# RicherMans/PLDA

Measured on AMD Instinct MI355X. Metric: PLDA LLR trials/sec, higher is better.
Workload: dtype f32; 1 GPU; C2: 100k i-vectors, featdim 200, 5k speakers; 100k x 100k trials, n = 1; fit 10 EM iters; D_eff=200; enrol_models=100000, test_vectors=100000, parallelism=one GPU, score_dtype=f32 (fp64 bias terms, fp32 MFMA contraction), fit_dtype=f64

## Files before the change

### plda_amd/csrc/eer.hip

```cpp
#include "trial_source.hpp"

#include <algorithm>
#include <cstring>

namespace plda {


typedef float f32x4e __attribute__((ext_vector_type(4)));

__global__ __launch_bounds__(256) void eer_hist_kernel(const float *__restrict__ scores, int64_t Nt, int fixed_class,
                                                       int shift, int nbits, unsigned prefix, int has_prefix,
                                                       unsigned long long *__restrict__ hist ,
                                                       unsigned *__restrict__ below, unsigned *__restrict__ above) {
  __shared__ unsigned lh[2][EER_BINS];
  for (int i = threadIdx.x; i < 2 * EER_BINS; i += 256) (&lh[0][0])[i] = 0;
  __syncthreads();
  const unsigned mask = (1u << nbits) - 1u;
  const int hi_shift = shift + nbits;
  unsigned lo_max = 0u, hi_min = 0xffffffffu;

  auto account = [&](bool ok, float sc, int cls) {
    unsigned bin = 0xffffffffu;
    if (ok) {
      const unsigned k = score_key(sc);
      if (has_prefix && (k >> hi_shift) != prefix) {
        if ((k >> hi_shift) < prefix) lo_max = k > lo_max ? k : lo_max; else hi_min = k < hi_min ? k : hi_min;
      } else {
        bin = ((k >> shift) & mask) | ((unsigned)cls << 11);
      }
    }
    if (bin != 0xffffffffu) atomicAdd(&lh[bin >> 11][bin & 2047u], 1u);
  };

  for (int64_t idx = (int64_t)blockIdx.x * 256 + threadIdx.x; idx - threadIdx.x < Nt; idx += (int64_t)gridDim.x * 256)
    account(idx < Nt, idx < Nt ? scores[idx] : 0.f, fixed_class);
  __syncthreads();
  for (int i = threadIdx.x; i < 2 * EER_BINS; i += 256) {
    const unsigned v = (&lh[0][0])[i];
    if (v) atomicAdd(hist + i, (unsigned long long)v);
  }
  if (has_prefix) {
    if (lo_max) atomicMax(below, lo_max);
    if (hi_min != 0xffffffffu) atomicMin(above, hi_min);
  }
}

__global__ __launch_bounds__(256) void eer_hist_strip_kernel(const float *__restrict__ scores, int64_t ld, int64_t M,
                                                             int64_t Nt, const int64_t *__restrict__ espk,
                                                             const int64_t *__restrict__ tspk, int64_t rows_per_wg,
                                                             int shift, int nbits, unsigned prefix, int has_prefix,
                                                             unsigned long long *__restrict__ hist,
                                                             unsigned *__restrict__ below, unsigned *__restrict__ above, int64_t row_step) {
  __shared__ unsigned lh[2][EER_BINS];
  for (int i = threadIdx.x; i < 2 * EER_BINS; i += 256) (&lh[0][0])[i] = 0;
  __syncthreads();
  const unsigned mask = (1u << nbits) - 1u;
  const int hi_shift = shift + nbits;
  unsigned lo_max = 0u, hi_min = 0xffffffffu;
  const int64_t strips = (Nt + EER_STRIP - 1) / EER_STRIP;
  const int64_t strip = blockIdx.x % strips, slice = blockIdx.x / strips;
  const int64_t col = strip * EER_STRIP + (int64_t)threadIdx.x * 4;
  const int64_t r0 = slice * rows_per_wg, r1 = (r0 + rows_per_wg < M) ? r0 + rows_per_wg : M;
  int64_t ts[4];
  bool ok[4];
#pragma unroll
  for (int e = 0; e < 4; ++e) {
    ok[e] = col + e < Nt;
    ts[e] = ok[e] ? tspk[col + e] : 0;
  }
  const bool vec = ((ld & 3) == 0) && ((reinterpret_cast<uintptr_t>(scores) & 15) == 0) && ok[3];

  auto account = [&](float sc, int cls) {
    const unsigned k = score_key(sc);
    if (has_prefix && (k >> hi_shift) != prefix) {
      if ((k >> hi_shift) < prefix) lo_max = k > lo_max ? k : lo_max; else hi_min = k < hi_min ? k : hi_min;
    } else {
      atomicAdd(&lh[cls][(k >> shift) & mask], 1u);
    }
  };

  for (int64_t row = r0; row < r1; row += 4) {
    float v[4][4];
#pragma unroll
    for (int u = 0; u < 4; ++u) {
      if (row + u >= r1) break;
      const float *src = scores + (row + u) * row_step * ld + col;
      if (vec) {
        const f32x4e x = __builtin_nontemporal_load(reinterpret_cast<const f32x4e *>(src));
        v[u][0] = x.x; v[u][1] = x.y; v[u][2] = x.z; v[u][3] = x.w;
      } else {
#pragma unroll
        for (int e = 0; e < 4; ++e) v[u][e] = ok[e] ? src[e] : 0.f;
      }
    }
#pragma unroll
    for (int u = 0; u < 4; ++u) {
      if (row + u >= r1) break;
      const int64_t spk = espk[(row + u) * row_step];
#pragma unroll
      for (int e = 0; e < 4; ++e) if (ok[e]) account(v[u][e], ts[e] == spk ? 1 : 0);
    }
  }
  __syncthreads();
  for (int i = threadIdx.x; i < 2 * EER_BINS; i += 256) {
    const unsigned c = (&lh[0][0])[i];
    if (c) atomicAdd(hist + i, (unsigned long long)c);
  }
  if (has_prefix) {
    if (lo_max) atomicMax(below, lo_max);
    if (hi_min != 0xffffffffu) atomicMin(above, hi_min);
  }
}

struct EerWindowOut {
  unsigned long long below[2], targets, above, cursor[2];
};
constexpr int EER_WBUF = 1536;
__global__ __launch_bounds__(256) void eer_window_strip_kernel(const float *__restrict__ scores, int64_t ld, int64_t M, int64_t Nt,
                                                               const int64_t *__restrict__ espk, const int64_t *__restrict__ tspk,
                                                               int64_t rows_per_wg, float flo, float fhi, EerWindowOut *__restrict__ wo,
                                                               float *__restrict__ list0, float *__restrict__ list1, unsigned long long cap) {
  __shared__ unsigned long long red[4][4];
  __shared__ float stage[4][2][EER_WBUF];
  __shared__ int fillc[4][2];
  const int64_t strips = (Nt + EER_STRIP - 1) / EER_STRIP;
  const int64_t strip = blockIdx.x % strips, slice = blockIdx.x / strips;
  const int64_t col = strip * EER_STRIP + (int64_t)threadIdx.x * 4;
  const int64_t r0 = slice * rows_per_wg, r1 = (r0 + rows_per_wg < M) ? r0 + rows_per_wg : M;
  const int lane = threadIdx.x & 63, wave = threadIdx.x >> 6;
  int64_t ts[4];
  bool ok[4];
#pragma unroll
  for (int e = 0; e < 4; ++e) {
    ok[e] = col + e < Nt;
    ts[e] = ok[e] ? tspk[col + e] : 0;
  }
  const bool vec = ((ld & 3) == 0) && ((reinterpret_cast<uintptr_t>(scores) & 15) == 0) && ok[3];
  const float qnan = __uint_as_float(0x7fc00000u);
  unsigned b0 = 0, b1 = 0, t1 = 0, ab = 0;
  int *const fc = fillc[wave];
  if (lane < 2) fc[lane] = 0;
  auto flush = [&](int c) {
    const int n = __builtin_amdgcn_readfirstlane(fc[c]);
    if (n == 0) return;
    unsigned long long base = 0;
    if (lane == 0) base = atomicAdd(&wo->cursor[c], (unsigned long long)n);
    base = __shfl(base, 0);
    float *dst = c ? list1 : list0;
    const float *src = stage[wave][c];
    for (int i = lane; i < n; i += 64)
      if (base + i < cap) dst[base + i] = src[i];
    if (lane == 0) fc[c] = 0;
  };
  for (int64_t row = r0; row < r1; row += 4) {
    float v[4][4];
#pragma unroll
    for (int u = 0; u < 4; ++u) {
      if (row + u >= r1) break;
      const float *src = scores + (row + u) * ld + col;
      if (vec) {
        const f32x4e x = __builtin_nontemporal_load(reinterpret_cast<const f32x4e *>(src));
        v[u][0] = x.x; v[u][1] = x.y; v[u][2] = x.z; v[u][3] = x.w;
      } else {
#pragma unroll
        for (int e = 0; e < 4; ++e) v[u][e] = ok[e] ? src[e] : qnan;
      }
    }
#pragma unroll
    for (int u = 0; u < 4; ++u) {
      if (row + u >= r1) break;
      const int64_t spk = espk[row + u];
#pragma unroll
      for (int e = 0; e < 4; ++e) {
        const float x = v[u][e];
        const bool tgt = ok[e] && ts[e] == spk;
        const bool lt_lo = x < flo, lt_hi = x < fhi;
        t1 += tgt ? 1u : 0u;
        b1 += (lt_lo && tgt) ? 1u : 0u;
        b0 += (lt_lo && !tgt) ? 1u : 0u;
        ab += (x >= fhi) ? 1u : 0u;
        if (lt_hi && !lt_lo) {
          const int c = tgt ? 1 : 0;
          const int slot = atomicAdd(&fc[c], 1);
          stage[wave][c][slot] = x;
        }
      }
    }
    if (__builtin_amdgcn_readfirstlane(fc[0]) > EER_WBUF - 1024) flush(0);
    if (__builtin_amdgcn_readfirstlane(fc[1]) > EER_WBUF - 1024) flush(1);
  }
  flush(0);
  flush(1);
  unsigned long long c[4] = {b0, b1, t1, ab};
#pragma unroll
  for (int q = 0; q < 4; ++q) {
    for (int o = 32; o > 0; o >>= 1) c[q] += __shfl_xor(c[q], o);
    if (lane == 0) red[wave][q] = c[q];
  }
  __syncthreads();
  if (threadIdx.x < 4) {
    const unsigned long long sum = (red[0][threadIdx.x] + red[1][threadIdx.x]) + (red[2][threadIdx.x] + red[3][threadIdx.x]);
    unsigned long long *dst = threadIdx.x == 0 ? &wo->below[0] : threadIdx.x == 1 ? &wo->below[1] : threadIdx.x == 2 ? &wo->targets : &wo->above;
    if (sum) atomicAdd(dst, sum);
  }
}


int eer_pass(plda_handle *h, const TrialSource &src, int shift, int nbits, unsigned prefix, int has_prefix,
             unsigned long long *dhist, unsigned *dbelow, unsigned *dabove, std::vector<unsigned long long> &hh) {
  PLDA_HIP(h, hipMemsetAsync(dhist, 0, 2 * EER_BINS * 8, h->stream));
  PLDA_TRY(for_each_piece(src, [&](const TrialPiece &pc) -> int {
    if (pc.cls < 0) {
      const int64_t strips = ceil_div(pc.Nt, (int64_t)EER_STRIP);
      const int64_t slices = std::max<int64_t>(1, std::min<int64_t>(pc.rows, (256 * 16) / strips));
      const int64_t rows_per_wg = ceil_div(pc.rows, slices);
      eer_hist_strip_kernel<<<(unsigned)(strips * ceil_div(pc.rows, rows_per_wg)), 256, 0, h->stream>>>(
          pc.scores, pc.ld, pc.rows, pc.Nt, pc.espk, src.tspk, rows_per_wg, shift, nbits, prefix, has_prefix, dhist, dbelow, dabove,
          pc.row_step);
    } else {
      const unsigned grid = (unsigned)std::min<int64_t>(ceil_div(pc.Nt, 256), 256 * 16);
      eer_hist_kernel<<<grid, 256, 0, h->stream>>>(pc.scores, pc.Nt, pc.cls, shift, nbits, prefix, has_prefix, dhist, dbelow, dabove);
    }
    return PLDA_OK;
  }));
  PLDA_LAUNCH_CHECK(h);
  hh.resize(2 * EER_BINS);
  PLDA_HIP(h, hipMemcpyAsync(hh.data(), dhist, 2 * EER_BINS * 8, hipMemcpyDeviceToHost, h->stream));
  PLDA_HIP(h, hipStreamSynchronize(h->stream));
  return PLDA_OK;
}

bool reduce_block_or_poison(plda_handle *h, const TrialSource &src, const char *who, unsigned long long *H, int *rc) {
  constexpr unsigned long long POISON = 1ull << 48;
  if (src.reduce) {
    if (*rc != PLDA_OK) { std::fill(H, H + 2 * EER_BINS, 0ull); H[0] = POISON; }
    if (src.reduce(src.ctx, H, nullptr, nullptr) != 0 && *rc == PLDA_OK) *rc = fail(h, PLDA_E_INVAL, "%s: the caller's reduction failed", who);
    if (*rc == PLDA_OK && H[0] >= POISON) *rc = fail(h, PLDA_E_NUMERIC, "%s: another rank of the sharded call failed", who);
  }
  return *rc == PLDA_OK;
}

static int eer_device(plda_handle *h, const TrialSource &src, double *out, bool *window_missed = nullptr) {
  typedef unsigned __int128 u128;
  if (window_missed) *window_missed = false;
  unsigned long long *dhist;
  unsigned *dbelow;
  PLDA_TRY(carve(h, h->trial_hist, [&](Layout &c) { c.take(dhist, 2 * EER_BINS).take(dbelow, 2).slack(56); }));
  unsigned *dabove = dbelow + 1;
  std::vector<unsigned long long> H;
  unsigned long long Np = 0, Nn = 0, Pb = 0, Nb = 0;
  unsigned prefix = 0;
  const int shifts[3] = {21, 10, 0}, bits[3] = {11, 11, 10};
  unsigned long long cP = 0, cN = 0;
  std::vector<unsigned long long> last;
  static const unsigned init[2] = {0u, 0xffffffffu};
  int rc = PLDA_OK;
  for (int pass = 0; pass < 3; ++pass) {
    if (rc == PLDA_OK && pass == 2) {
      const hipError_t e = hipMemcpyAsync(dbelow, init, 8, hipMemcpyHostToDevice, h->stream);
      if (e != hipSuccess) rc = hip_fail(h, e, "hipMemcpyAsync(dbelow)", __FILE__, __LINE__);
    }
    if (rc == PLDA_OK) rc = eer_pass(h, src, shifts[pass], bits[pass], prefix, pass > 0, dhist, dbelow, dabove, H);
    H.resize(2 * EER_BINS);
    if (!reduce_block_or_poison(h, src, "eer", H.data(), &rc)) continue;
    const int nb = 1 << bits[pass];
    if (pass == 0) {
      for (int b = 0; b < nb; ++b) { Nn += H[b]; Np += H[EER_BINS + b]; }
      if (src.windowed) { Np = src.tot_p; Nn = src.tot_n; Pb = src.base_p; Nb = src.base_n; }
      if (Np == 0 || Nn == 0) { rc = fail(h, PLDA_E_INVAL, "eer: need at least one target and one impostor trial"); continue; }
    }
    int sel = -1;
    unsigned long long P = Pb, N = Nb;
    for (int b = 0; b < nb; ++b) {
      const unsigned long long p2 = P + H[EER_BINS + b], n2 = N + H[b];
      if ((H[b] | H[EER_BINS + b]) && (u128)p2 * Nn >= (u128)(Nn - n2) * Np) { sel = b; cP = H[EER_BINS + b]; cN = H[b]; break; }
      P = p2; N = n2;
    }
    if (sel < 0 && src.windowed && window_missed) { *window_missed = true; return PLDA_OK; }
    if (sel < 0) { rc = fail(h, PLDA_E_NUMERIC, "eer: crossing not found (inconsistent counts)"); continue; }
    Pb = P; Nb = N;
    prefix = (prefix << bits[pass]) | (unsigned)sel;
    if (pass == 2) last = H;
  }
  unsigned hb[2] = {0u, 0xffffffffu};
  if (rc == PLDA_OK) {
    hipError_t e = hipMemcpyAsync(hb, dbelow, 8, hipMemcpyDeviceToHost, h->stream);
    if (e == hipSuccess) e = hipStreamSynchronize(h->stream);
    if (e != hipSuccess) rc = hip_fail(h, e, "copy of the neighbour keys", __FILE__, __LINE__);
  }
  if (src.reduce && src.reduce(src.ctx, nullptr, &hb[0], &hb[1]) != 0 && rc == PLDA_OK)
    rc = fail(h, PLDA_E_INVAL, "eer: the caller's reduction failed");
  if (rc != PLDA_OK) return rc;
  const unsigned k1 = prefix;
  const int b2 = (int)(k1 & 1023u);
  long long k0 = -1, k2 = -1;
  for (int b = b2 - 1; b >= 0; --b) if (last[b] | last[EER_BINS + b]) { k0 = (long long)((k1 & ~1023u) | (unsigned)b); break; }
  if (k0 < 0 && (Pb + Nb) > 0) k0 = hb[0];
  for (int b = b2 + 1; b < 1024; ++b) if (last[b] | last[EER_BINS + b]) { k2 = (long long)((k1 & ~1023u) | (unsigned)b); break; }
  if (k2 < 0 && (Pb + cP + Nb + cN) < (Np + Nn)) k2 = hb[1];
  if (src.windowed) {
    const bool need0 = (Pb + Nb) > 0, need2 = (Pb + cP + Nb + cN) < (Np + Nn);
    if ((need0 && k0 == 0) || (need2 && k2 == 0xffffffffll)) { if (window_missed) *window_missed = true; return PLDA_OK; }
  }
  const double far1 = (double)(Nn - Nb - cN) / (double)Nn, frr1 = (double)(Pb + cP) / (double)Np;
  const double far0 = (double)(Nn - Nb) / (double)Nn, frr0 = (double)Pb / (double)Np;
  double thr, far, frr;
  if (fabs(far1 - frr1) <= fabs(far0 - frr0)) {
    const double s = key_score(k1);
    thr = k2 >= 0 ? s + ((double)key_score((unsigned)k2) - s) / 2.0 : s + 1e-8;
    far = (double)(Nn - Nb - cN) / (double)Nn; frr = (double)(Pb + cP) / (double)Np;
  } else {
    const double s1 = key_score(k1);
    thr = k0 >= 0 ? (double)key_score((unsigned)k0) + (s1 - (double)key_score((unsigned)k0)) / 2.0 : s1;
    far = (double)(Nn - Nb) / (double)Nn; frr = (double)Pb / (double)Np;
  }
  out[0] = thr; out[1] = far; out[2] = frr; out[3] = 0.5 * (far + frr); out[4] = (double)Np; out[5] = (double)Nn;
  return PLDA_OK;
}

constexpr int64_t EER_PILOT_STEP = 32;
static int eer_matrix_windowed(plda_handle *h, const TrialSource &full, double *out, bool *done) {
  typedef unsigned __int128 u128;
  *done = false;
  const int64_t M = full.M, Nt = full.Nt;
  TraceScope ts(h, "eer.pilot");
  unsigned long long *dhist;
  unsigned *dbelow;
  EerWindowOut *dwo;
  PLDA_TRY(carve(h, h->trial_hist, [&](Layout &c) { c.take(dhist, 2 * EER_BINS).take(dbelow, 2).take(dwo, 1, 64); }));
  unsigned *dabove = dbelow + 1;
  TrialSource smp = TrialSource::matrix(full.scores, full.ld, M, Nt, full.espk, full.tspk).every(EER_PILOT_STEP);
  int64_t pilot_step = EER_PILOT_STEP;
  if (full.kind == TrialSource::SLABS) {
    pilot_step = std::max<int64_t>(EER_PILOT_STEP, ceil_div(M, full.sl->slab_rows));
    const float *sc = nullptr; const int64_t *se = nullptr; int64_t sld = 0, srows = 0;
    PLDA_TRY(full.sl->sample(full.sl->ctx, pilot_step, &sc, &sld, &se, &srows));
    smp = TrialSource::matrix(sc, sld, srows, Nt, se, full.tspk);
  }
  std::vector<unsigned long long> H0, H1;
  PLDA_TRY(eer_pass(h, smp, 21, 11, 0, 0, dhist, dbelow, dabove, H0));
  unsigned long long Np = 0, Nn = 0;
  for (int b = 0; b < EER_BINS; ++b) { Nn += H0[b]; Np += H0[EER_BINS + b]; }
  if (Np < 2000 || Nn < 2000) return PLDA_OK;
  auto g_after = [&](unsigned long long p, unsigned long long n) { return (double)p / (double)Np - (double)(Nn - n) / (double)Nn; };
  double delta = 0.0;
  {
    unsigned long long P = 0, N = 0;
    int c0 = -1;
    for (int b = 0; b < EER_BINS; ++b) {
      const unsigned long long p2 = P + H0[EER_BINS + b], n2 = N + H0[b];
      if ((H0[b] | H0[EER_BINS + b]) && (u128)p2 * Nn >= (u128)(Nn - n2) * Np) { c0 = b; break; }
      P = p2; N = n2;
    }
    if (c0 < 0) return PLDA_OK;
    const double pe = std::min(0.5, std::max((double)P / (double)Np, 10.0 / (double)Np));
    delta = 5.0 * (std::sqrt(pe * (1.0 - pe) / (double)Np) + std::sqrt(pe * (1.0 - pe) / (double)Nn)) + 2.0 / (double)Np;
  }
  int ca = -1, cb = -1;
  unsigned long long Pa = 0, Na = 0, Pc = 0, Nc = 0;
  {
    unsigned long long P = 0, N = 0;
    for (int b = 0; b < EER_BINS; ++b) {
      const unsigned long long p2 = P + H0[EER_BINS + b], n2 = N + H0[b];
      const double g = g_after(p2, n2);
      if (ca < 0 && g > -delta) { ca = b; Pa = P; Na = N; }
      if (g >= delta) { cb = b; Pc = P; Nc = N; break; }
      P = p2; N = n2;
    }
  }
  if (ca < 0 || cb < 0) return PLDA_OK;
  int blo = 0, bhi = EER_BINS - 1;
  unsigned long long win_lo = Pa + Na, win_hi = 0;
  PLDA_TRY(eer_pass(h, smp, 10, 11, (unsigned)ca, 1, dhist, dbelow, dabove, H1));
  {
    unsigned long long p = Pa, n = Na;
    for (int b = 0; b < EER_BINS; ++b) {
      const unsigned long long p2 = p + H1[EER_BINS + b], n2 = n + H1[b];
      if (g_after(p2, n2) > -delta) { blo = b; break; }
      p = p2; n = n2;
    }
    blo = std::max(blo - 1, 0);
    for (int b = 0; b < blo; ++b) win_lo += H1[b] + H1[EER_BINS + b];
  }
  if (cb != ca) PLDA_TRY(eer_pass(h, smp, 10, 11, (unsigned)cb, 1, dhist, dbelow, dabove, H1));
  {
    unsigned long long p = Pc, n = Nc;
    for (int b = 0; b < EER_BINS; ++b) {
      p += H1[EER_BINS + b]; n += H1[b];
      if (g_after(p, n) >= delta) { bhi = b; break; }
    }
    bhi = std::min(bhi + 1, EER_BINS - 1);
    win_hi = Pc + Nc;
    for (int b = 0; b <= bhi; ++b) win_hi += H1[b] + H1[EER_BINS + b];
  }
  const unsigned klo = ((unsigned)ca << 21) | ((unsigned)blo << 10);
  const unsigned long long khi64 = ((unsigned long long)cb << 21) | ((unsigned long long)(bhi + 1) << 10);
  if (khi64 > 0xffffffffull || khi64 <= klo) return PLDA_OK;
  const unsigned khi = (unsigned)khi64;
  const unsigned long long win = win_hi > win_lo ? win_hi - win_lo : 0;
  const unsigned long long cap = (unsigned long long)((double)win * (double)pilot_step * 2.0) + (1ull << 20);
  if (cap > (unsigned long long)M * (unsigned long long)Nt / 8) return PLDA_OK;
  PLDA_HIP(h, h->eer_list[0].reserve((size_t)cap * 4));
  PLDA_HIP(h, h->eer_list[1].reserve((size_t)cap * 4));
  ts.next("eer.window_pass", (double)M * (double)Nt * 4.0, 2);
  PLDA_HIP(h, hipMemsetAsync(dwo, 0, sizeof(EerWindowOut), h->stream));
  PLDA_TRY(for_each_piece(full, [&](const TrialPiece &pc) -> int {
    const int64_t strips = ceil_div(Nt, (int64_t)EER_STRIP);
    const int64_t slices = std::max<int64_t>(1, std::min<int64_t>(pc.rows, (256 * 16) / strips));
    const int64_t rows_per_wg = ceil_div(pc.rows, slices);
    eer_window_strip_kernel<<<(unsigned)(strips * ceil_div(pc.rows, rows_per_wg)), 256, 0, h->stream>>>(
        pc.scores, pc.ld, pc.rows, Nt, pc.espk, full.tspk, rows_per_wg, key_score(klo), key_score(khi), dwo, h->eer_list[0].as<float>(), h->eer_list[1].as<float>(), cap);
    PLDA_LAUNCH_CHECK(h);
    return PLDA_OK;
  }));
  EerWindowOut wo;
  PLDA_HIP(h, hipMemcpyAsync(&wo, dwo, sizeof(wo), hipMemcpyDeviceToHost, h->stream));
  PLDA_HIP(h, hipStreamSynchronize(h->stream));
  ts.next("eer.finish_on_window");
  if (wo.cursor[0] > cap || wo.cursor[1] > cap) return PLDA_OK;
  if (wo.below[0] + wo.below[1] + wo.cursor[0] + wo.cursor[1] + wo.above != (unsigned long long)M * (unsigned long long)Nt) return PLDA_OK;
  const unsigned long long TP = wo.targets, TN = (unsigned long long)M * (unsigned long long)Nt - wo.targets;
  if (TP == 0 || TN == 0) return fail(h, PLDA_E_INVAL, "eer: need at least one target and one impostor trial");
  if ((u128)wo.below[1] * TN >= (u128)(TN - wo.below[0]) * TP) return PLDA_OK;
  if ((u128)(wo.below[1] + wo.cursor[1]) * TN < (u128)(TN - wo.below[0] - wo.cursor[0]) * TP) return PLDA_OK;
  if (wo.cursor[0] + wo.cursor[1] == 0) return PLDA_OK;
  const TrialSource lst = TrialSource::lists(h->eer_list[1].as<float>(), (int64_t)wo.cursor[1], h->eer_list[0].as<float>(), (int64_t)wo.cursor[0])
                              .window_of(wo.below[1], wo.below[0], TP, TN);
  bool missed = false;
  PLDA_TRY(eer_device(h, lst, out, &missed));
  *done = !missed;
  return PLDA_OK;
}

static int eer_source_device(plda_handle *h, const TrialSource &src, double *out, const char *three_passes_scope) {
  const int64_t M = src.M, Nt = src.Nt;
  h->eer_last_passes = 3;
  if (!src.reduce && h->eer_variant != 1 && (h->eer_variant == 2 || (double)M * (double)Nt >= 2.5e8) && M >= 4 * EER_PILOT_STEP) {
    bool done = false;
    PLDA_TRY(eer_matrix_windowed(h, src, out, &done));
    if (done) { h->eer_last_passes = 1; return PLDA_OK; }
  }
  TraceScope ts(h, three_passes_scope, 3.0 * (double)M * (double)Nt * 4.0, 2);
  return eer_device(h, src, out);
}

int eer_matrix_device(plda_handle *h, const float *dscores, int64_t ld, int64_t M, int64_t Nt, const int64_t *despk,
                      const int64_t *dtspk, double *out, TrialReduce reduce, void *ctx) {
  if (!out || Nt <= 0 || ld < Nt || M < 0 || (M == 0 && !reduce) || (M > 0 && (!dscores || !despk || !dtspk)))
    return fail(h, PLDA_E_INVAL, "eer: bad argument");
  return eer_source_device(h, TrialSource::matrix(dscores, ld, M, Nt, despk, dtspk).reduced_by(reduce, ctx), out, "eer.three_passes");
}

int score_eer_device(plda_handle *h, const double *dU, const int32_t *dn, int n_uniform, int64_t M, const double *dV, int64_t Nt,
                     const double *dzmean, const double *dzstd, const int64_t *despk, const int64_t *dtspk, double *out) {
  OperandSlabs os;
  TrialSource src;
  PLDA_TRY(operand_source(h, "score_eer", dU, dn, n_uniform, M, dV, Nt, dzmean, dzstd, despk, dtspk, out, &os, &src));
  return eer_source_device(h, src, out, "eer.three_passes (slabs re-scored per pass)");
}

constexpr int DET_MAX = 2047;
__global__ __launch_bounds__(256) void det_minmax_kernel(const float *__restrict__ scores, int64_t ld, int64_t M, int64_t Nt,
                                                         unsigned *__restrict__ mm ) {
  unsigned lo = 0xffffffffu, hi = 0u;
  const int64_t total = M * Nt;
  for (int64_t idx = (int64_t)blockIdx.x * 256 + threadIdx.x; idx < total; idx += (int64_t)gridDim.x * 256) {
    const unsigned k = score_key(scores[(idx / Nt) * ld + idx % Nt]);
    lo = k < lo ? k : lo; hi = k > hi ? k : hi;
  }
  for (int o = 32; o > 0; o >>= 1) {
    const unsigned a = __shfl_xor(lo, o), b = __shfl_xor(hi, o);
    lo = a < lo ? a : lo; hi = b > hi ? b : hi;
  }
  if ((threadIdx.x & 63) == 0) { atomicMin(mm, lo); atomicMax(mm + 1, hi); }
}
__global__ __launch_bounds__(256) void det_hist_kernel(const float *__restrict__ scores, int64_t ld, int64_t M, int64_t Nt,
                                                       const int64_t *__restrict__ espk, const int64_t *__restrict__ tspk, int cls,
                                                       const double *__restrict__ thr, int n, double lo, double inv_step,
                                                       unsigned long long *__restrict__ hist ) {
  __shared__ unsigned lh[2][DET_MAX + 1];
  __shared__ double ts[DET_MAX + 1];
  for (int i = threadIdx.x; i < 2 * (DET_MAX + 1); i += 256) (&lh[0][0])[i] = 0;
  for (int i = threadIdx.x; i < n; i += 256) ts[i] = thr[i];
  __syncthreads();
  const int64_t total = M * Nt;
  for (int64_t idx = (int64_t)blockIdx.x * 256 + threadIdx.x; idx < total; idx += (int64_t)gridDim.x * 256) {
    const int64_t r = idx / Nt, c = idx % Nt;
    const double sc = (double)scores[r * ld + c];
    int k = (int)((sc - lo) * inv_step) + 1;
    k = k < 0 ? 0 : (k > n ? n : k);
    while (k > 0 && ts[k - 1] > sc) --k;
    while (k < n && ts[k] <= sc) ++k;
    const int cl = cls >= 0 ? cls : (espk[r] == tspk[c] ? 1 : 0);
    atomicAdd(&lh[cl][k], 1u);
  }
  __syncthreads();
  for (int i = threadIdx.x; i < 2 * (DET_MAX + 1); i += 256) {
    const unsigned v = (&lh[0][0])[i];
    if (v) atomicAdd(hist + i, (unsigned long long)v);
  }
}

static int det_device(plda_handle *h, const TrialSource &src, int npoints, double *far, double *frr, double *thresholds) {
  if (npoints < 2 || npoints > DET_MAX) return fail(h, PLDA_E_INVAL, "det: 2 <= n_points <= %d", DET_MAX);
  const size_t hb = (size_t)2 * (DET_MAX + 1) * 8;
  unsigned long long *dhist;
  unsigned *dmm;
  double *dthr;
  PLDA_TRY(carve(h, h->trial_hist, [&](Layout &c) { c.take(dhist, 2 * (DET_MAX + 1)).take(dmm, 16).take(dthr, DET_MAX).slack(64); }));
  static const unsigned init[2] = {0xffffffffu, 0u};
  PLDA_HIP(h, hipMemcpyAsync(dmm, init, 8, hipMemcpyHostToDevice, h->stream));
  PLDA_TRY(for_each_piece(src, [&](const TrialPiece &pc) -> int {
    det_minmax_kernel<<<(unsigned)std::min<int64_t>(ceil_div(pc.rows * pc.Nt, 256), 256 * 32), 256, 0, h->stream>>>(pc.scores, pc.ld, pc.rows, pc.Nt, dmm);
    return PLDA_OK;
  }));
  PLDA_LAUNCH_CHECK(h);
  unsigned mm[2];
  PLDA_HIP(h, hipMemcpyAsync(mm, dmm, 8, hipMemcpyDeviceToHost, h->stream));
  PLDA_HIP(h, hipStreamSynchronize(h->stream));
  if (mm[0] > mm[1]) return fail(h, PLDA_E_INVAL, "det: no scores");
  const double lo = (double)key_score(mm[0]), hi = (double)key_score(mm[1]);
  const double step = (hi - lo) / ((double)npoints - 1.0);
  std::vector<double> thr((size_t)npoints);
  double t = lo;
  for (int i = 0; i < npoints; ++i) { thr[(size_t)i] = t; t += step; }
  PLDA_HIP(h, hipMemcpyAsync(dthr, thr.data(), (size_t)npoints * 8, hipMemcpyHostToDevice, h->stream));
  PLDA_HIP(h, hipMemsetAsync(dhist, 0, hb, h->stream));
  PLDA_TRY(for_each_piece(src, [&](const TrialPiece &pc) -> int {
    det_hist_kernel<<<(unsigned)std::min<int64_t>(ceil_div(pc.rows * pc.Nt, 256), 256 * 8), 256, 0, h->stream>>>(
        pc.scores, pc.ld, pc.rows, pc.Nt, pc.espk, src.tspk, pc.cls, dthr, npoints, lo, step > 0.0 ? 1.0 / step : 0.0, dhist);
    return PLDA_OK;
  }));
  PLDA_LAUNCH_CHECK(h);
  std::vector<unsigned long long> H((size_t)2 * (DET_MAX + 1));
  PLDA_HIP(h, hipMemcpyAsync(H.data(), dhist, hb, hipMemcpyDeviceToHost, h->stream));
  PLDA_HIP(h, hipStreamSynchronize(h->stream));
  unsigned long long Nn = 0, Np = 0;
  for (int k = 0; k <= npoints; ++k) { Nn += H[(size_t)k]; Np += H[(size_t)(DET_MAX + 1) + k]; }
  if (Nn == 0 || Np == 0) return fail(h, PLDA_E_INVAL, "det: need at least one target and one impostor score");
  unsigned long long below_p = 0, ge_n = Nn;
  for (int i = 0; i < npoints; ++i) {
    ge_n -= H[(size_t)i];
    below_p += H[(size_t)(DET_MAX + 1) + i];
    far[i] = (double)ge_n / (double)Nn;
    frr[i] = (double)below_p / (double)Np;
    if (thresholds) thresholds[i] = thr[(size_t)i];
  }
  return PLDA_OK;
}

int det_matrix_device(plda_handle *h, const float *dscores, int64_t ld, int64_t M, int64_t Nt, const int64_t *despk, const int64_t *dtspk,
                      int npoints, double *far, double *frr, double *thresholds) {
  if (!dscores || !despk || !dtspk || !far || !frr || M <= 0 || Nt <= 0 || ld < Nt) return fail(h, PLDA_E_INVAL, "det: bad argument");
  return det_device(h, TrialSource::matrix(dscores, ld, M, Nt, despk, dtspk), npoints, far, frr, thresholds);
}
int det_lists_device(plda_handle *h, const float *dpos, int64_t np, const float *dneg, int64_t nn, int npoints, double *far, double *frr,
                     double *thresholds) {
  if (!dpos || !dneg || !far || !frr || np <= 0 || nn <= 0) return fail(h, PLDA_E_INVAL, "det: need at least one target and one impostor score");
  return det_device(h, TrialSource::lists(dpos, np, dneg, nn), npoints, far, frr, thresholds);
}

int eer_lists_device(plda_handle *h, const float *dpos, int64_t np, const float *dneg, int64_t nn, double *out) {
  if (!dpos || !dneg || !out || np <= 0 || nn <= 0) return fail(h, PLDA_E_INVAL, "eer: need at least one target and one impostor score");
  return eer_device(h, TrialSource::lists(dpos, np, dneg, nn), out);
}

}
```

Before: 363.7 billion trials/s.

## Move windowed EER refinement on-device and rebalance window pass with persistent grid

The window pass becomes a persistent kernel sized to resident occupancy, with fixed row-chunk work units spread evenly over blocks. LDS stage-slot atomics are replaced by wave ballots and prefix popcounts. The per-pass host readback in the windowed list refinement is replaced by a single-block device scan kernel that chains the three histogram passes and reads back once. Neighbour min/max atomics are reduced per wave and skipped when they cannot change the stored value. This removes host sync round-trips and contention, at the cost of more kernel complexity and a smaller staging buffer that flushes more often.

```diff
diff --git a/plda_amd/csrc/eer.hip b/plda_amd/csrc/eer.hip
--- a/plda_amd/csrc/eer.hip
+++ b/plda_amd/csrc/eer.hip
@@ -7,14 +7,29 @@
 
 
 typedef float f32x4e __attribute__((ext_vector_type(4)));
+
+__device__ __forceinline__ void neighbours_to_global(unsigned lo_max, unsigned hi_min, unsigned *__restrict__ below,
+                                                     unsigned *__restrict__ above) {
+  for (int o = 32; o > 0; o >>= 1) {
+    const unsigned a = __shfl_xor(lo_max, o), b = __shfl_xor(hi_min, o);
+    lo_max = a > lo_max ? a : lo_max;
+    hi_min = b < hi_min ? b : hi_min;
+  }
+  if ((threadIdx.x & 63) == 0) {
+    if (lo_max > __hip_atomic_load(below, __ATOMIC_RELAXED, __HIP_MEMORY_SCOPE_AGENT)) atomicMax(below, lo_max);
+    if (hi_min < __hip_atomic_load(above, __ATOMIC_RELAXED, __HIP_MEMORY_SCOPE_AGENT)) atomicMin(above, hi_min);
+  }
+}
 
 __global__ __launch_bounds__(256) void eer_hist_kernel(const float *__restrict__ scores, int64_t Nt, int fixed_class,
                                                        int shift, int nbits, unsigned prefix, int has_prefix,
                                                        unsigned long long *__restrict__ hist ,
-                                                       unsigned *__restrict__ below, unsigned *__restrict__ above) {
+                                                       unsigned *__restrict__ below, unsigned *__restrict__ above,
+                                                       const unsigned *__restrict__ dprefix = nullptr) {
   __shared__ unsigned lh[2][EER_BINS];
   for (int i = threadIdx.x; i < 2 * EER_BINS; i += 256) (&lh[0][0])[i] = 0;
   __syncthreads();
+  if (dprefix) prefix = *dprefix;
   const unsigned mask = (1u << nbits) - 1u;
   const int hi_shift = shift + nbits;
   unsigned lo_max = 0u, hi_min = 0xffffffffu;
@@ -39,10 +54,7 @@
     const unsigned v = (&lh[0][0])[i];
     if (v) atomicAdd(hist + i, (unsigned long long)v);
   }
-  if (has_prefix) {
-    if (lo_max) atomicMax(below, lo_max);
-    if (hi_min != 0xffffffffu) atomicMin(above, hi_min);
-  }
+  if (has_prefix) neighbours_to_global(lo_max, hi_min, below, above);
 }
 
 __global__ __launch_bounds__(256) void eer_hist_strip_kernel(const float *__restrict__ scores, int64_t ld, int64_t M,
@@ -106,42 +118,30 @@
     const unsigned c = (&lh[0][0])[i];
     if (c) atomicAdd(hist + i, (unsigned long long)c);
   }
-  if (has_prefix) {
-    if (lo_max) atomicMax(below, lo_max);
-    if (hi_min != 0xffffffffu) atomicMin(above, hi_min);
-  }
+  if (has_prefix) neighbours_to_global(lo_max, hi_min, below, above);
 }
 
 struct EerWindowOut {
   unsigned long long below[2], targets, above, cursor[2];
 };
-constexpr int EER_WBUF = 1536;
+constexpr int EER_WROWS = 8;
+constexpr int EER_WROW_MAX = 256;
+constexpr int EER_WBUF = 512;
+static_assert(EER_WBUF >= 2 * EER_WROW_MAX, "a row must fit the stage behind the flush threshold");
 __global__ __launch_bounds__(256) void eer_window_strip_kernel(const float *__restrict__ scores, int64_t ld, int64_t M, int64_t Nt,
                                                                const int64_t *__restrict__ espk, const int64_t *__restrict__ tspk,
-                                                               int64_t rows_per_wg, float flo, float fhi, EerWindowOut *__restrict__ wo,
-                                                               float *__restrict__ list0, float *__restrict__ list1, unsigned long long cap) {
-  __shared__ unsigned long long red[4][4];
+                                                               int64_t chunks, int64_t units, float flo, float fhi, EerWindowOut *__restrict__ wo,
+                                                               float *__restrict__ list0, float *__restrict__ list1, unsigned long long cap,
+                                                               unsigned long long *__restrict__ hist_clear) {
   __shared__ float stage[4][2][EER_WBUF];
-  __shared__ int fillc[4][2];
-  const int64_t strips = (Nt + EER_STRIP - 1) / EER_STRIP;
-  const int64_t strip = blockIdx.x % strips, slice = blockIdx.x / strips;
-  const int64_t col = strip * EER_STRIP + (int64_t)threadIdx.x * 4;
-  const int64_t r0 = slice * rows_per_wg, r1 = (r0 + rows_per_wg < M) ? r0 + rows_per_wg : M;
+  if (hist_clear && blockIdx.x == 0)
+    for (int i = threadIdx.x; i < 2 * EER_BINS; i += 256) hist_clear[i] = 0ull;
   const int lane = threadIdx.x & 63, wave = threadIdx.x >> 6;
-  int64_t ts[4];
-  bool ok[4];
-#pragma unroll
-  for (int e = 0; e < 4; ++e) {
-    ok[e] = col + e < Nt;
-    ts[e] = ok[e] ? tspk[col + e] : 0;
-  }
-  const bool vec = ((ld & 3) == 0) && ((reinterpret_cast<uintptr_t>(scores) & 15) == 0) && ok[3];
+  const unsigned long long lower = (1ull << lane) - 1ull;
   const float qnan = __uint_as_float(0x7fc00000u);
-  unsigned b0 = 0, b1 = 0, t1 = 0, ab = 0;
-  int *const fc = fillc[wave];
-  if (lane < 2) fc[lane] = 0;
-  auto flush = [&](int c) {
-    const int n = __builtin_amdgcn_readfirstlane(fc[c]);
+  unsigned wlo = 0, wlo1 = 0, wt = 0, wab = 0;
+  int fill0 = 0, fill1 = 0;
+  auto flush = [&](int c, int n) {
     if (n == 0) return;
     unsigned long long base = 0;
     if (lane == 0) base = atomicAdd(&wo->cursor[c], (unsigned long long)n);
@@ -150,56 +150,73 @@
     const float *src = stage[wave][c];
     for (int i = lane; i < n; i += 64)
       if (base + i < cap) dst[base + i] = src[i];
-    if (lane == 0) fc[c] = 0;
   };
-  for (int64_t row = r0; row < r1; row += 4) {
-    float v[4][4];
-#pragma unroll
-    for (int u = 0; u < 4; ++u) {
-      if (row + u >= r1) break;
-      const float *src = scores + (row + u) * ld + col;
-      if (vec) {
-        const f32x4e x = __builtin_nontemporal_load(reinterpret_cast<const f32x4e *>(src));
-        v[u][0] = x.x; v[u][1] = x.y; v[u][2] = x.z; v[u][3] = x.w;
-      } else {
-#pragma unroll
-        for (int e = 0; e < 4; ++e) v[u][e] = ok[e] ? src[e] : qnan;
-      }
-    }
-#pragma unroll
-    for (int u = 0; u < 4; ++u) {
-      if (row + u >= r1) break;
-      const int64_t spk = espk[row + u];
-#pragma unroll
-      for (int e = 0; e < 4; ++e) {
-        const float x = v[u][e];
-        const bool tgt = ok[e] && ts[e] == spk;
-        const bool lt_lo = x < flo, lt_hi = x < fhi;
-        t1 += tgt ? 1u : 0u;
-        b1 += (lt_lo && tgt) ? 1u : 0u;
-        b0 += (lt_lo && !tgt) ? 1u : 0u;
-        ab += (x >= fhi) ? 1u : 0u;
-        if (lt_hi && !lt_lo) {
-          const int c = tgt ? 1 : 0;
-          const int slot = atomicAdd(&fc[c], 1);
-          stage[wave][c][slot] = x;
+  const int64_t u_end = units * ((int64_t)blockIdx.x + 1) / gridDim.x;
+  for (int64_t u0 = units * (int64_t)blockIdx.x / gridDim.x; u0 < u_end;) {
+    const int64_t strip = u0 / chunks, c0 = u0 % chunks;
+    const int64_t c1 = (c0 + (u_end - u0) < chunks) ? c0 + (u_end - u0) : chunks;
+    const int64_t r0 = c0 * EER_WROWS, r1 = (c1 * EER_WROWS < M) ? c1 * EER_WROWS : M;
+    u0 += c1 - c0;
+    const int64_t col = strip * EER_STRIP + (int64_t)threadIdx.x * 4;
+    int64_t ts[4];
+    bool ok[4];
+#pragma unroll
+    for (int e = 0; e < 4; ++e) {
+      ok[e] = col + e < Nt;
+      ts[e] = ok[e] ? tspk[col + e] : 0;
+    }
+    const bool vec = ((ld & 3) == 0) && ((reinterpret_cast<uintptr_t>(scores) & 15) == 0) && ok[3];
+    for (int64_t row = r0; row < r1; row += 4) {
+      float v[4][4];
+#pragma unroll
+      for (int u = 0; u < 4; ++u) {
+        if (row + u >= r1) break;
+        const float *src = scores + (row + u) * ld + col;
+        if (vec) {
+          const f32x4e x = __builtin_nontemporal_load(reinterpret_cast<const f32x4e *>(src));
+          v[u][0] = x.x; v[u][1] = x.y; v[u][2] = x.z; v[u][3] = x.w;
+        } else {
+#pragma unroll
+          for (int e = 0; e < 4; ++e) v[u][e] = ok[e] ? src[e] : qnan;
         }
       }
-    }
-    if (__builtin_amdgcn_readfirstlane(fc[0]) > EER_WBUF - 1024) flush(0);
-    if (__builtin_amdgcn_readfirstlane(fc[1]) > EER_WBUF - 1024) flush(1);
-  }
-  flush(0);
-  flush(1);
-  unsigned long long c[4] = {b0, b1, t1, ab};
-#pragma unroll
-  for (int q = 0; q < 4; ++q) {
-    for (int o = 32; o > 0; o >>= 1) c[q] += __shfl_xor(c[q], o);
-    if (lane == 0) red[wave][q] = c[q];
-  }
+#pragma unroll
+      for (int u = 0; u < 4; ++u) {
+        if (row + u >= r1) break;
+        const int64_t spk = espk[row + u];
+#pragma unroll
+        for (int e = 0; e < 4; ++e) {
+          const float x = v[u][e];
+          const bool tgt = ok[e] && ts[e] == spk, lt_lo = x < flo, lt_hi = x < fhi;
+          wt += tgt ? 1u : 0u;
+          wlo += lt_lo ? 1u : 0u;
+          wlo1 += (lt_lo && tgt) ? 1u : 0u;
+          wab += (x >= fhi) ? 1u : 0u;
+          const unsigned long long mt = __ballot(tgt), mlo = __ballot(lt_lo), mhi = __ballot(lt_hi);
+          const unsigned long long m = mhi & ~mlo;
+          if (m) {
+            const unsigned long long m1 = m & mt, m0 = m ^ m1;
+            if (lt_hi && !lt_lo) stage[wave][tgt ? 1 : 0][tgt ? fill1 + __popcll(m1 & lower) : fill0 + __popcll(m0 & lower)] = x;
+            fill0 += __popcll(m0);
+            fill1 += __popcll(m1);
+          }
+        }
+        if (fill0 > EER_WBUF - EER_WROW_MAX) { flush(0, fill0); fill0 = 0; }
+        if (fill1 > EER_WBUF - EER_WROW_MAX) { flush(1, fill1); fill1 = 0; }
+      }
+    }
+  }
+  flush(0, fill0);
+  flush(1, fill1);
+  unsigned long long *const red = reinterpret_cast<unsigned long long *>(&stage[wave][0][0]);
+  unsigned long long c[4] = {wlo - wlo1, wlo1, wt, wab};
+#pragma unroll
+  for (int q = 0; q < 4; ++q) for (int o = 32; o > 0; o >>= 1) c[q] += __shfl_xor(c[q], o);
+  if (lane == 0) { red[0] = c[0]; red[1] = c[1]; red[2] = c[2]; red[3] = c[3]; }
   __syncthreads();
   if (threadIdx.x < 4) {
-    const unsigned long long sum = (red[0][threadIdx.x] + red[1][threadIdx.x]) + (red[2][threadIdx.x] + red[3][threadIdx.x]);
+    unsigned long long sum = 0;
+    for (int w = 0; w < 4; ++w) sum += reinterpret_cast<const unsigned long long *>(&stage[w][0][0])[threadIdx.x];
     unsigned long long *dst = threadIdx.x == 0 ? &wo->below[0] : threadIdx.x == 1 ? &wo->below[1] : threadIdx.x == 2 ? &wo->targets : &wo->above;
     if (sum) atomicAdd(dst, sum);
   }
@@ -240,9 +257,10 @@
   return *rc == PLDA_OK;
 }
 
-static int eer_device(plda_handle *h, const TrialSource &src, double *out, bool *window_missed = nullptr) {
+static bool eer_result(bool windowed, unsigned long long Np, unsigned long long Nn, unsigned long long Pb, unsigned long long Nb,
+                       unsigned long long cP, unsigned long long cN, unsigned k1, int b0, int b3, const unsigned *hb, double *out);
+static int eer_device(plda_handle *h, const TrialSource &src, double *out) {
   typedef unsigned __int128 u128;
-  if (window_missed) *window_missed = false;
   unsigned long long *dhist;
   unsigned *dbelow;
   PLDA_TRY(carve(h, h->trial_hist, [&](Layout &c) { c.take(dhist, 2 * EER_BINS).take(dbelow, 2).slack(56); }));
@@ -266,7 +284,6 @@
     const int nb = 1 << bits[pass];
     if (pass == 0) {
       for (int b = 0; b < nb; ++b) { Nn += H[b]; Np += H[EER_BINS + b]; }
-      if (src.windowed) { Np = src.tot_p; Nn = src.tot_n; Pb = src.base_p; Nb = src.base_n; }
       if (Np == 0 || Nn == 0) { rc = fail(h, PLDA_E_INVAL, "eer: need at least one target and one impostor trial"); continue; }
     }
     int sel = -1;
@@ -276,7 +293,6 @@
       if ((H[b] | H[EER_BINS + b]) && (u128)p2 * Nn >= (u128)(Nn - n2) * Np) { sel = b; cP = H[EER_BINS + b]; cN = H[b]; break; }
       P = p2; N = n2;
     }
-    if (sel < 0 && src.windowed && window_missed) { *window_missed = true; return PLDA_OK; }
     if (sel < 0) { rc = fail(h, PLDA_E_NUMERIC, "eer: crossing not found (inconsistent counts)"); continue; }
     Pb = P; Nb = N;
     prefix = (prefix << bits[pass]) | (unsigned)sel;
@@ -293,14 +309,21 @@
   if (rc != PLDA_OK) return rc;
   const unsigned k1 = prefix;
   const int b2 = (int)(k1 & 1023u);
-  long long k0 = -1, k2 = -1;
-  for (int b = b2 - 1; b >= 0; --b) if (last[b] | last[EER_BINS + b]) { k0 = (long long)((k1 & ~1023u) | (unsigned)b); break; }
+  int b0 = -1, b3 = -1;
+  for (int b = b2 - 1; b >= 0; --b) if (last[b] | last[EER_BINS + b]) { b0 = b; break; }
+  for (int b = b2 + 1; b < 1024; ++b) if (last[b] | last[EER_BINS + b]) { b3 = b; break; }
+  (void)eer_result(false, Np, Nn, Pb, Nb, cP, cN, k1, b0, b3, hb, out);
+  return PLDA_OK;
+}
+
+static bool eer_result(bool windowed, unsigned long long Np, unsigned long long Nn, unsigned long long Pb, unsigned long long Nb,
+                       unsigned long long cP, unsigned long long cN, unsigned k1, int b0, int b3, const unsigned *hb, double *out) {
+  long long k0 = b0 >= 0 ? (long long)((k1 & ~1023u) | (unsigned)b0) : -1, k2 = b3 >= 0 ? (long long)((k1 & ~1023u) | (unsigned)b3) : -1;
   if (k0 < 0 && (Pb + Nb) > 0) k0 = hb[0];
-  for (int b = b2 + 1; b < 1024; ++b) if (last[b] | last[EER_BINS + b]) { k2 = (long long)((k1 & ~1023u) | (unsigned)b); break; }
   if (k2 < 0 && (Pb + cP + Nb + cN) < (Np + Nn)) k2 = hb[1];
-  if (src.windowed) {
+  if (windowed) {
     const bool need0 = (Pb + Nb) > 0, need2 = (Pb + cP + Nb + cN) < (Np + Nn);
-    if ((need0 && k0 == 0) || (need2 && k2 == 0xffffffffll)) { if (window_missed) *window_missed = true; return PLDA_OK; }
+    if ((need0 && k0 == 0) || (need2 && k2 == 0xffffffffll)) return false;
   }
   const double far1 = (double)(Nn - Nb - cN) / (double)Nn, frr1 = (double)(Pb + cP) / (double)Np;
   const double far0 = (double)(Nn - Nb) / (double)Nn, frr0 = (double)Pb / (double)Np;
@@ -315,6 +338,112 @@
     far = (double)(Nn - Nb) / (double)Nn; frr = (double)Pb / (double)Np;
   }
   out[0] = thr; out[1] = far; out[2] = frr; out[3] = 0.5 * (far + frr); out[4] = (double)Np; out[5] = (double)Nn;
+  return true;
+}
+
+struct EerRefine {
+  unsigned long long Np, Nn;
+  unsigned long long Pb, Nb;
+  unsigned long long cP, cN;
+  unsigned prefix;
+  int failed;
+  int b0, b3;
+  unsigned below, above;
+};
+__device__ __forceinline__ bool prod_ge(unsigned long long a, unsigned long long b, unsigned long long c, unsigned long long d) {
+  const unsigned long long h1 = __umul64hi(a, b), l1 = a * b, h2 = __umul64hi(c, d), l2 = c * d;
+  return h1 > h2 || (h1 == h2 && l1 >= l2);
+}
+__global__ __launch_bounds__(256) void eer_refine_scan_kernel(unsigned long long *__restrict__ hist, EerRefine *__restrict__ st, int pass,
+                                                              int nbits, int first, EerRefine init) {
+  constexpr int PER = EER_BINS / 256;
+  __shared__ unsigned long long sp[4], sn[4];
+  __shared__ int ssel, slo, shi;
+  const int t = threadIdx.x, lane = t & 63, wave = t >> 6;
+  unsigned long long p[PER], n[PER], tp = 0, tn = 0;
+#pragma unroll
+  for (int i = 0; i < PER; ++i) {
+    n[i] = hist[t * PER + i];
+    p[i] = hist[EER_BINS + t * PER + i];
+    tp += p[i]; tn += n[i];
+  }
+  unsigned long long ip = tp, in = tn;
+  for (int o = 1; o < 64; o <<= 1) {
+    const unsigned long long a = __shfl_up(ip, o), b = __shfl_up(in, o);
+    if (lane >= o) { ip += a; in += b; }
+  }
+  if (lane == 63) { sp[wave] = ip; sn[wave] = in; }
+  if (t == 0) { ssel = EER_BINS; slo = -1; shi = EER_BINS; }
+  const EerRefine s = first ? init : *st;
+  __syncthreads();
+  unsigned long long P = s.Pb + (ip - tp), N = s.Nb + (in - tn);
+  for (int w = 0; w < wave; ++w) { P += sp[w]; N += sn[w]; }
+  int mine = -1;
+  unsigned long long Pm = 0, Nm = 0, cPm = 0, cNm = 0;
+#pragma unroll
+  for (int i = 0; i < PER; ++i) {
+    const unsigned long long p2 = P + p[i], n2 = N + n[i];
+    if (mine < 0 && (p[i] | n[i]) && prod_ge(p2, s.Nn, s.Nn - n2, s.Np)) { mine = t * PER + i; Pm = P; Nm = N; cPm = p[i]; cNm = n[i]; }
+    P = p2; N = n2;
+  }
+  if (mine >= 0) atomicMin(&ssel, mine);
+  __syncthreads();
+  const int sel = ssel;
+  if (pass == 2 && sel < EER_BINS) {
+#pragma unroll
+    for (int i = 0; i < PER; ++i) {
+      const int b = t * PER + i;
+      if (p[i] | n[i]) {
+        if (b < sel) atomicMax(&slo, b);
+        if (b > sel) atomicMin(&shi, b);
+      }
+    }
+  }
+  __syncthreads();
+  if (sel == EER_BINS) {
+    if (t == 0) {
+      EerRefine r = s;
+      if (r.failed < 0) r.failed = pass;
+      *st = r;
+    }
+  } else if (mine == sel) {
+    EerRefine r = s;
+    r.Pb = Pm; r.Nb = Nm; r.cP = cPm; r.cN = cNm;
+    r.prefix = (s.prefix << nbits) | (unsigned)sel;
+    if (pass == 2) { r.b0 = slo; r.b3 = shi < EER_BINS ? shi : -1; }
+    else { r.below = 0u; r.above = 0xffffffffu; }
+    *st = r;
+  }
+  if (pass < 2) {
+#pragma unroll
+    for (int i = 0; i < PER; ++i) { hist[t * PER + i] = 0ull; hist[EER_BINS + t * PER + i] = 0ull; }
+  }
+}
+
+static int eer_window_lists_device(plda_handle *h, const TrialSource &lst, int coarse, unsigned long long *dhist, EerRefine *dst, double *out,
+                                   bool *missed) {
+  *missed = false;
+  const int shifts[3] = {21, 10, 0}, bits[3] = {11, 11, 10};
+  EerRefine st{};
+  st.Np = lst.tot_p; st.Nn = lst.tot_n; st.Pb = lst.base_p; st.Nb = lst.base_n;
+  st.failed = -1; st.b0 = st.b3 = -1; st.below = 0u; st.above = 0xffffffffu;
+  int first = 1;
+  if (coarse >= 0) { st.cP = (unsigned long long)lst.np; st.cN = (unsigned long long)lst.nn; st.prefix = (unsigned)coarse; }
+  for (int pass = coarse >= 0 ? 1 : 0; pass < 3; ++pass) {
+    PLDA_TRY(for_each_piece(lst, [&](const TrialPiece &pc) -> int {
+      const unsigned grid = (unsigned)std::min<int64_t>(ceil_div(pc.Nt, 256), 256 * 16);
+      eer_hist_kernel<<<grid, 256, 0, h->stream>>>(pc.scores, pc.Nt, pc.cls, shifts[pass], bits[pass], st.prefix, pass > 0, dhist, &dst->below,
+                                                   &dst->above, first ? nullptr : &dst->prefix);
+      return PLDA_OK;
+    }));
+    eer_refine_scan_kernel<<<1, 256, 0, h->stream>>>(dhist, dst, pass, bits[pass], first, st);
+    first = 0;
+  }
+  PLDA_LAUNCH_CHECK(h);
+  PLDA_HIP(h, hipMemcpyAsync(&st, dst, sizeof(st), hipMemcpyDeviceToHost, h->stream));
+  PLDA_HIP(h, hipStreamSynchronize(h->stream));
+  const unsigned hb[2] = {st.below, st.above};
+  *missed = st.failed >= 0 || !eer_result(true, st.Np, st.Nn, st.Pb, st.Nb, st.cP, st.cN, st.prefix, st.b0, st.b3, hb, out);
   return PLDA_OK;
 }
 
@@ -327,7 +456,8 @@
   unsigned long long *dhist;
   unsigned *dbelow;
   EerWindowOut *dwo;
-  PLDA_TRY(carve(h, h->trial_hist, [&](Layout &c) { c.take(dhist, 2 * EER_BINS).take(dbelow, 2).take(dwo, 1, 64); }));
+  EerRefine *dst;
+  PLDA_TRY(carve(h, h->trial_hist, [&](Layout &c) { c.take(dhist, 2 * EER_BINS).take(dbelow, 2).take(dwo, 1, 64).take(dst, 1, 64).slack(48); }));
   unsigned *dabove = dbelow + 1;
   TrialSource smp = TrialSource::matrix(full.scores, full.ld, M, Nt, full.espk, full.tspk).every(EER_PILOT_STEP);
   int64_t pilot_step = EER_PILOT_STEP;
@@ -399,24 +529,29 @@
   const unsigned khi = (unsigned)khi64;
   const unsigned long long win = win_hi > win_lo ? win_hi - win_lo : 0;
   const unsigned long long cap = (unsigned long long)((double)win * (double)pilot_step * 2.0) + (1ull << 20);
-  if (cap > (unsigned long long)M * (unsigned long long)Nt / 8) return PLDA_OK;
+  if (h->eer_variant != 2 && cap > (unsigned long long)M * (unsigned long long)Nt / 8) return PLDA_OK;
   PLDA_HIP(h, h->eer_list[0].reserve((size_t)cap * 4));
   PLDA_HIP(h, h->eer_list[1].reserve((size_t)cap * 4));
   ts.next("eer.window_pass", (double)M * (double)Nt * 4.0, 2);
   PLDA_HIP(h, hipMemsetAsync(dwo, 0, sizeof(EerWindowOut), h->stream));
+  int per_cu = 0;
+  PLDA_HIP(h, hipOccupancyMaxActiveBlocksPerMultiprocessor(&per_cu, eer_window_strip_kernel, 256, 0));
+  const int64_t resident = (int64_t)std::max(per_cu, 1) * std::max(h->num_cus, 1);
+  bool first_piece = true;
   PLDA_TRY(for_each_piece(full, [&](const TrialPiece &pc) -> int {
-    const int64_t strips = ceil_div(Nt, (int64_t)EER_STRIP);
-    const int64_t slices = std::max<int64_t>(1, std::min<int64_t>(pc.rows, (256 * 16) / strips));
-    const int64_t rows_per_wg = ceil_div(pc.rows, slices);
-    eer_window_strip_kernel<<<(unsigned)(strips * ceil_div(pc.rows, rows_per_wg)), 256, 0, h->stream>>>(
-        pc.scores, pc.ld, pc.rows, Nt, pc.espk, full.tspk, rows_per_wg, key_score(klo), key_score(khi), dwo, h->eer_list[0].as<float>(), h->eer_list[1].as<float>(), cap);
+    const int64_t strips = ceil_div(Nt, (int64_t)EER_STRIP), chunks = ceil_div(pc.rows, (int64_t)EER_WROWS);
+    const int64_t units = strips * chunks;
+    eer_window_strip_kernel<<<(unsigned)std::min(units, resident), 256, 0, h->stream>>>(
+        pc.scores, pc.ld, pc.rows, Nt, pc.espk, full.tspk, chunks, units, key_score(klo), key_score(khi), dwo, h->eer_list[0].as<float>(),
+        h->eer_list[1].as<float>(), cap, first_piece ? dhist : nullptr);
+    first_piece = false;
     PLDA_LAUNCH_CHECK(h);
     return PLDA_OK;
   }));
   EerWindowOut wo;
   PLDA_HIP(h, hipMemcpyAsync(&wo, dwo, sizeof(wo), hipMemcpyDeviceToHost, h->stream));
   PLDA_HIP(h, hipStreamSynchronize(h->stream));
-  ts.next("eer.finish_on_window");
+  ts.next("eer.finish_on_window", (double)(wo.cursor[0] + wo.cursor[1]));
   if (wo.cursor[0] > cap || wo.cursor[1] > cap) return PLDA_OK;
   if (wo.below[0] + wo.below[1] + wo.cursor[0] + wo.cursor[1] + wo.above != (unsigned long long)M * (unsigned long long)Nt) return PLDA_OK;
   const unsigned long long TP = wo.targets, TN = (unsigned long long)M * (unsigned long long)Nt - wo.targets;
@@ -427,7 +562,7 @@
   const TrialSource lst = TrialSource::lists(h->eer_list[1].as<float>(), (int64_t)wo.cursor[1], h->eer_list[0].as<float>(), (int64_t)wo.cursor[0])
                               .window_of(wo.below[1], wo.below[0], TP, TN);
   bool missed = false;
-  PLDA_TRY(eer_device(h, lst, out, &missed));
+  PLDA_TRY(eer_window_lists_device(h, lst, ca == cb ? ca : -1, dhist, dst, out, &missed));
   *done = !missed;
   return PLDA_OK;
 }
```

Result: no change. 363.9 billion trials/s, median of 4 (+0.1%).
